# tj12323/GeoPurify

Hardware: AMD Instinct MI355X
Metric: scenes/sec (ScanNet-val shape) + pooled-feature GB/s vs HBM peak (higher is better)
Workload: dtype f32 (student convolutions and pooling: f16 hi/lo split operands, 3 MFMAs per product, fp32 accumulate)

## Files before the change

### geopurify_amd/_lib.py

```python
import ctypes
import os
from ctypes import POINTER, c_char_p, c_double, c_float, c_int32, c_int64, c_size_t, c_uint32, c_uint64, c_void_p

_HERE = os.path.dirname(os.path.abspath(__file__))
LIB_PATH = os.environ.get("GP_LIB") or os.path.join(_HERE, "libgeopurify_hip.so")

_P = c_void_p
GP_KNN_MAX_K = 127
GP_KNN_QUERY_MAX_K = 32
GP_ELEM_F32, GP_ELEM_F16, GP_ELEM_BF16 = 0, 1, 2
GP_LABEL_U8, GP_LABEL_I16, GP_LABEL_I32, GP_LABEL_I64 = 0, 1, 2, 3

SIGNATURES = {
    "gp_version": (c_int32, []),
    "gp_last_error": (c_char_p, []),
    "gp_debug_set": (c_int32, [c_int32, c_int32]),
    "gp_debug_ptr": (c_int32, [c_int32, _P, c_size_t]),
    "gp_voxelize_workspace_bytes": (c_size_t, [c_int64]),
    "gp_voxelize_f64": (c_int32, [_P, c_int64, POINTER(c_double), _P, _P, _P, _P, _P, _P, _P, c_size_t, _P]),
    "gp_fnv_hash_f64": (c_int32, [_P, c_int64, _P, _P]),
    "gp_project_points_f64": (c_int32, [_P, c_int64, POINTER(c_double), c_double, c_double, c_double,
                                        c_double, _P, c_int32, c_int32, c_int32, c_double, _P, _P, _P]),
    "gp_render_depth_f64": (c_int32, [_P, c_int64, POINTER(c_double), c_double, c_double, c_double, c_double,
                                      c_int32, c_int32, c_int32, _P, _P]),
# ... 69 lines not shown
    "gp_pool_cs_chain_flag_words": (c_size_t, [c_int64, c_int32]),
    "gp_pool_cs_chain_flag_words_d": (c_size_t, [c_int64, c_int32, c_int32]),
    "gp_pool_cs_apply_chain": (c_int32, [_P, _P, _P, _P, c_int64, _P, _P, _P, _P, _P, c_int64, c_int32, c_int32, c_int32, _P, c_int64, _P, _P, _P,
                                         c_uint32, _P]),
    "gp_lift_dense_accum": (c_int32, [_P, c_int32, c_int32, c_int32, _P, _P, _P, c_int64, _P, c_int64, _P, _P]),
    "gp_lift_dense_bilinear_accum": (c_int32, [_P, c_int32, c_int32, c_int32, c_int32, c_int32, _P, _P, _P, c_int64, _P,
                                               c_int64, _P, _P]),
    "gp_lift_dense_finish": (c_int32, [_P, c_int64, c_int32, _P, c_int64, _P, _P]),
    "gp_lift_masks_workspace_bytes": (c_size_t, [c_int32, c_int32, c_int32]),
    "gp_lift_masks_view": (c_int32, [_P, c_int32, c_int32, c_int32, _P, _P, _P, _P, _P, c_int32, c_int32,
                                     _P, _P, c_int64, _P, _P, _P, c_size_t, _P]),
    "gp_pv_count": (c_int32, [_P, c_int64, _P, _P]),
    "gp_scan_workspace_bytes": (c_size_t, [c_int64]),
    "gp_exclusive_scan_i64": (c_int32, [_P, c_int64, _P, _P, c_size_t, _P]),
    "gp_pv_fill": (c_int32, [_P, _P, c_int64, c_int32, _P, _P, _P, _P, _P]),
    "gp_segment_tables": (c_int32, [_P, c_int32, c_int32, _P, c_int32, c_float, _P, _P, _P]),
    "gp_fuse_views_top3": (c_int32, [_P, _P, _P, c_int64, _P, _P, c_int32, c_int32, c_int32, _P, c_int64, _P, _P]),
    "gp_seen_masks": (c_int32, [_P, c_int64, _P, _P, _P]),
    "gp_fuse_views_top3_fill": (c_int32, [_P, _P, _P, c_int64, _P, _P, c_int32, c_int32, c_int32, _P, _P, c_int64, _P]),
    "gp_nn1_workspace_bytes": (c_size_t, [c_int64, c_int64]),
    "gp_nn1_f64": (c_int32, [_P, c_int64, _P, c_int64, _P, _P, c_size_t, _P]),
    "gp_nn1_masked_workspace_bytes": (c_size_t, [c_int64]),
    "gp_nn1_masked_f64": (c_int32, [_P, c_int64, _P, _P, _P, _P, c_size_t, _P]),
    "gp_visible_lists_workspace_bytes": (c_size_t, [c_int64]),
    "gp_visible_lists": (c_int32, [_P, c_int64, _P, _P, _P, _P, _P, c_size_t, _P]),
    "gp_views_visible_lists_workspace_bytes": (c_size_t, [c_int64, c_int32]),
    "gp_views_visible_lists": (c_int32, [_P, c_int64, _P, _P, c_int32, c_int32, c_int32, c_int32, c_double, c_int64, c_int64,
                                         _P, _P, _P, _P, _P, _P, _P, c_size_t, _P]),
    "gp_lift_masks_views_workspace_bytes": (c_size_t, [c_int32, c_int32, c_int32, c_int32, c_int64, c_int64, c_int64]),
    "gp_lift_masks_views": (c_int32, [_P, c_int32, c_int32, c_int32, c_int32, _P, _P, _P, _P, _P, c_int32, c_int32, _P, c_int64,
                                      _P, _P, _P, _P, _P, _P, c_int32, c_int64, c_int64, _P, _P, _P, _P, _P, c_size_t, _P]),
    "gp_classify_argmax": (c_int32, [_P, c_int64, c_int32, c_int64, _P, c_int32, c_float, _P, _P, _P]),
    "gp_gather_rows_classify": (c_int32, [_P, c_int64, c_int32, _P, c_int64, _P, _P, c_int64, _P, c_int32, c_float, _P, _P, _P]),
    "gp_rows_argmax": (c_int32, [_P, c_int64, c_int32, c_int64, _P, c_int64, c_int32, _P, _P, _P]),
    "gp_col_stats_workspace_bytes": (c_size_t, [c_int64, c_int32]),
    "gp_col_stats": (c_int32, [_P, c_int64, c_int64, c_int32, _P, _P, _P, c_size_t, _P]),
    "gp_bn_train_apply": (c_int32, [_P, c_int64, c_int64, c_int32, _P, _P, _P, _P, c_float, _P, c_int64, c_int32, _P, c_int64,
                                    _P, _P, c_int64, c_float, _P, _P, _P]),
    "gp_bn_train_backward_workspace_bytes": (c_size_t, [c_int64, c_int32]),
    "gp_bn_train_backward": (c_int32, [_P, c_int64, _P, c_int64, _P, c_int64, _P, _P, c_float, _P, _P, c_int64, c_int32, _P, c_int64,
                                       _P, c_int64, _P, _P, _P, _P, _P, c_int64, _P, c_size_t, _P]),
    "gp_col_sums_f64": (c_int32, [_P, c_int64, c_int64, c_int32, _P, _P, _P, c_size_t, _P]),
    "gp_bn_bwd_sums_f64": (c_int32, [_P, c_int64, _P, c_int64, _P, c_int64, _P, _P, c_float, _P, _P, c_int64, c_int32, _P, _P, c_size_t, _P]),
    "gp_bn_bwd_apply": (c_int32, [_P, c_int64, _P, c_int64, _P, c_int64, _P, _P, c_float, _P, _P, _P, c_int64, c_int64, c_int32, _P, c_int64,
                                  _P, c_int64, _P, _P]),
    "gp_infonce_workspace_bytes": (c_size_t, [c_int64, c_int32]),
    "gp_infonce_fwd_bwd": (c_int32, [_P, c_int64, c_int64, c_int32, _P, c_int64, _P, c_int64, c_int32, c_float, _P, _P, c_int64,
                                     _P, c_size_t, _P]),
    "gp_infonce_weighted_fwd_bwd": (c_int32, [_P, c_int64, c_int64, c_int32, _P, c_int64, _P, c_int64, c_int32, c_float, _P, _P, _P, _P, c_int64,
                                              _P, c_size_t, _P]),
    "gp_conv_wgrad_workspace_bytes": (c_size_t, [c_int64, c_int32, c_int32]),
    "gp_conv_wgrad_f16x3": (c_int32, [_P, _P, c_int64, _P, _P, c_int64, _P, _P, _P, c_int64, _P, c_int32, c_int32, c_int32, c_int32,
                                      _P, _P, _P, c_size_t, _P]),
    "gp_adamw_step": (c_int32, [_P, _P, _P, _P, c_int64, c_float, c_float, c_float, c_float, c_float, c_int64, _P]),
    "gp_knn_points_f32": (c_int32, [_P, c_int64, _P, c_int64, c_int32, _P, _P, _P]),
    "gp_sampler_select": (c_int32, [_P, c_int64, c_int64, c_int64, _P, c_int32, _P, _P, _P]),
    "gp_sim_segments_f16x3": (c_int32, [_P, _P, c_int64, c_int32, _P, _P, _P, _P, c_int64, c_int64, _P, _P]),
    "gp_sampler_select_segments": (c_int32, [_P, _P, _P, _P, c_int64, c_int64, _P, c_int32, _P, _P, _P]),
    "gp_sampler_micro_segments": (c_int32, [_P, _P, _P, _P, _P, c_int64, c_int32, _P, c_int64, c_int32, _P, _P]),
    "gp_normalize_split_f16": (c_int32, [_P, c_int64, c_int32, c_int64, c_int64, c_float, _P, _P, c_int64, _P]),
    "gp_iou_hist_i64": (c_int32, [_P, _P, c_int64, c_int32, POINTER(c_int64), c_int32, _P, _P]),
    "gp_nn1_batched_workspace_bytes": (c_size_t, [c_int64]),
    "gp_nn1_batched": (c_int32, [_P, _P, _P, _P, c_int64, c_int32, _P, _P, _P, c_size_t, _P]),
    "gp_iou_hist_batched_i64": (c_int32, [_P, _P, c_int64, _P, _P, c_int64, c_int32, c_int32, POINTER(c_int64), c_int32, _P, _P]),
    "gp_sparse_conv_tiles": (c_int32, [POINTER(c_int32)]),
    "gp_segment_loss_col_step": (c_int32, []),
# ... 142 lines not shown
```

### geopurify_amd/csrc/misc.hip

```cpp
#include <cstring>
#include <rocprim/device/device_scan.hpp>

#include "gp_common.h"
#include "gp_scan_bytes.h"

namespace {

constexpr int NN_TILE = 1024;

__global__ void __launch_bounds__(256)
nn1_partial_kernel(const float *__restrict__ ref, int64_t n_ref, const float *__restrict__ qry, int64_t n_q,
                   int splits, double *__restrict__ pd, int64_t *__restrict__ pi) {
    __shared__ double sx[NN_TILE], sy[NN_TILE], sz[NN_TILE];
    int64_t q = blockIdx.x * (int64_t)blockDim.x + threadIdx.x;
    int sp = blockIdx.y;
    int64_t per = (n_ref + splits - 1) / splits;
    int64_t r0 = sp * per, r1 = r0 + per < n_ref ? r0 + per : n_ref;
    double qx = 0, qy = 0, qz = 0;
    if (q < n_q) { qx = qry[q * 3]; qy = qry[q * 3 + 1]; qz = qry[q * 3 + 2]; }
    double best = INFINITY;
    int64_t bi = -1;
    for (int64_t t0 = r0; t0 < r1; t0 += NN_TILE) {
        int64_t cnt = r1 - t0 < NN_TILE ? r1 - t0 : NN_TILE;
        __syncthreads();
// ... 320 lines not shown
    for (int j = 0; j < CL_MAXJ; ++j) {
        v[j] = (live && j < nj) ? *reinterpret_cast<const float4 *>(feat + p * ld + (j * 16 + l) * 4) : make_float4(0.f, 0.f, 0.f, 0.f);
        ss += v[j].x * v[j].x + v[j].y * v[j].y + v[j].z * v[j].z + v[j].w * v[j].w;
    }
    ss = sum16(ss);
    const float nrm = fmaxf(sqrtf(ss), 1e-12f);
    float sa = 0.f;
#pragma unroll
    for (int j = 0; j < CL_MAXJ; ++j) {
        v[j].x /= nrm; v[j].y /= nrm; v[j].z /= nrm; v[j].w /= nrm;
        sa += fabsf(v[j].x) + fabsf(v[j].y) + fabsf(v[j].z) + fabsf(v[j].w);
    }
    sa = sum16(sa);
    float bestv = -INFINITY;
    int bestc = 0;
    for (int k = 0; k < C; ++k) {
        float dot = 0.f;
#pragma unroll
        for (int j = 0; j < CL_MAXJ; ++j)
            if (j < nj) {
                const float4 t = *reinterpret_cast<const float4 *>(text + (int64_t)k * d + (j * 16 + l) * 4);
                dot += v[j].x * t.x + v[j].y * t.y + v[j].z * t.z + v[j].w * t.w;
            }
        dot = sum16(dot) * scale;
        if (dot > bestv) { bestv = dot; bestc = k; }
    }
    if (live && l == 0) {
        pred[p] = bestc;
        if (zero_row) zero_row[p] = (sa == 0.f) ? 1 : 0;
    }
}

constexpr int CL_Q = 2;
template <bool GATHER>
__global__ void __launch_bounds__(256)
classify16_lds_kernel(const float *__restrict__ feat, int64_t ld, int d, int64_t n, const float *__restrict__ text, int C,
                      float scale, int64_t *__restrict__ pred, uint8_t *__restrict__ zero_row, const int64_t *__restrict__ index,
                      const int32_t *__restrict__ row_map, float *__restrict__ out, int64_t ld_out) {
    extern __shared__ __align__(16) float cl_text[];
    for (int i = threadIdx.x * 4; i < C * d; i += 256 * 4) *reinterpret_cast<float4 *>(cl_text + i) = *reinterpret_cast<const float4 *>(text + i);
    __syncthreads();
    const int l = threadIdx.x & 15, g = threadIdx.x >> 4;
    const int nj = d / 64;
    for (int64_t base = blockIdx.x * (int64_t)(16 * CL_Q); base < n; base += (int64_t)gridDim.x * (16 * CL_Q)) {
        float4 v[CL_Q][CL_MAXJ];
        float sa[CL_Q], bestv[CL_Q];
        int bestc[CL_Q];
        bool live[CL_Q];
#pragma unroll
        for (int q = 0; q < CL_Q; ++q) {
            const int64_t p = base + g * CL_Q + q;
            live[q] = p < n;
            int64_t src_row = p;
            if constexpr (GATHER) {
                if (live[q]) { src_row = index[p]; if (row_map) src_row = row_map[src_row]; }
            }
            float ss = 0.f;
#pragma unroll
            for (int j = 0; j < CL_MAXJ; ++j) {
                v[q][j] = (live[q] && j < nj) ? *reinterpret_cast<const float4 *>(feat + src_row * ld + (j * 16 + l) * 4) : make_float4(0.f, 0.f, 0.f, 0.f);
                if constexpr (GATHER) {
                    if (live[q] && j < nj) *reinterpret_cast<float4 *>(out + p * ld_out + (j * 16 + l) * 4) = v[q][j];
                }
                ss += v[q][j].x * v[q][j].x + v[q][j].y * v[q][j].y + v[q][j].z * v[q][j].z + v[q][j].w * v[q][j].w;
            }
            ss = sum16(ss);
            const float nrm = fmaxf(sqrtf(ss), 1e-12f);
            float a = 0.f;
#pragma unroll
            for (int j = 0; j < CL_MAXJ; ++j) {
                v[q][j].x /= nrm; v[q][j].y /= nrm; v[q][j].z /= nrm; v[q][j].w /= nrm;
                a += fabsf(v[q][j].x) + fabsf(v[q][j].y) + fabsf(v[q][j].z) + fabsf(v[q][j].w);
            }
            sa[q] = sum16(a);
            bestv[q] = -INFINITY;
            bestc[q] = 0;
        }
        for (int k = 0; k < C; ++k) {
            float dot[CL_Q];
#pragma unroll
            for (int q = 0; q < CL_Q; ++q) dot[q] = 0.f;
#pragma unroll
            for (int j = 0; j < CL_MAXJ; ++j)
                if (j < nj) {
                    const float4 t = *reinterpret_cast<const float4 *>(cl_text + k * d + (j * 16 + l) * 4);
#pragma unroll
                    for (int q = 0; q < CL_Q; ++q) dot[q] += v[q][j].x * t.x + v[q][j].y * t.y + v[q][j].z * t.z + v[q][j].w * t.w;
                }
#pragma unroll
            for (int q = 0; q < CL_Q; ++q) {
                const float dv = sum16(dot[q]) * scale;
                if (dv > bestv[q]) { bestv[q] = dv; bestc[q] = k; }
            }
        }
#pragma unroll
        for (int q = 0; q < CL_Q; ++q)
            if (live[q] && l == 0) {
                const int64_t p = base + g * CL_Q + q;
                pred[p] = bestc[q];
                if (zero_row) zero_row[p] = (sa[q] == 0.f) ? 1 : 0;
            }
    }
}

constexpr int CL_WJ = 16;
__global__ void __launch_bounds__(256)
classify_wave_gather_kernel(const float *__restrict__ feat, int64_t ld, int d, int64_t n, const float *__restrict__ text, int C,
                            float scale, int64_t *__restrict__ pred, uint8_t *__restrict__ zero_row, const int64_t *__restrict__ index,
                            const int32_t *__restrict__ row_map, float *__restrict__ out, int64_t ld_out) {
    extern __shared__ __align__(16) float cl_text[];
    for (int i = threadIdx.x * 4; i < C * d; i += 256 * 4) *reinterpret_cast<float4 *>(cl_text + i) = *reinterpret_cast<const float4 *>(text + i);
    __syncthreads();
    const int lane = threadIdx.x & 63, w = threadIdx.x >> 6;
    const int nj = d / 64;
    for (int64_t base = blockIdx.x * (int64_t)(4 * CL_Q); base < n; base += (int64_t)gridDim.x * (4 * CL_Q)) {
        float u[CL_Q][CL_WJ];
        float sa[CL_Q], bestv[CL_Q];
        int bestc[CL_Q];
        bool live[CL_Q];
#pragma unroll
        for (int q = 0; q < CL_Q; ++q) {
            const int64_t p = base + w * CL_Q + q;
            live[q] = p < n;
            int64_t src_row = 0;
            if (live[q]) { src_row = index[p]; if (row_map) src_row = row_map[src_row]; }
            float ss = 0.f;
#pragma unroll
            for (int j = 0; j < CL_WJ; ++j) {
                u[q][j] = (live[q] && j < nj) ? feat[src_row * ld + j * 64 + lane] : 0.f;
                if (live[q] && j < nj) out[p * ld_out + j * 64 + lane] = u[q][j];
                ss += u[q][j] * u[q][j];
            }
            ss = gp_wave_sum(ss);
            const float nrm = fmaxf(sqrtf(ss), 1e-12f);
// ... 253 lines not shown
    } else if (fast)
        classify16_kernel<<<(int)((n * 16 + 255) / 256), 256, 0, gp_stream(stream_)>>>(feat, ld, d, n, text_norm, c, logit_scale, pred, zero_row);
    else
        classify_kernel<<<(int)((n * 64 + 255) / 256), 256, 0, gp_stream(stream_)>>>(feat, ld, d, n, text_norm, c, logit_scale,
                                                                                   pred, zero_row);
    GP_CHECK_LAUNCH();
    return GP_OK;
}

extern "C" int gp_gather_rows_classify(const float *src, int64_t ld_src, int32_t d, const int64_t *index, int64_t n, const int32_t *row_map,
                                       float *out, int64_t ld_out, const float *text_norm, int32_t c, float logit_scale, int64_t *pred,
                                       uint8_t *zero_row, void *stream_) {
    GP_CHECK_ARG(src && index && out && text_norm && pred && n > 0 && d > 0 && c > 0, "gp_gather_rows_classify: null/empty argument");
    GP_CHECK_ARG(d % 64 == 0 && d <= 64 * CL_WJ && ld_src % 4 == 0 && ld_out % 4 == 0 && ld_out >= d && (uintptr_t)src % 16 == 0 &&
                     (uintptr_t)out % 16 == 0 && (uintptr_t)text_norm % 16 == 0 && (size_t)c * d * sizeof(float) <= 64 * 1024,
                 "gp_gather_rows_classify: d=%d must be a multiple of 64 up to %d, rows 16-byte aligned, c * d * 4 <= 64 KiB (use gp_gather_rows + "
                 "gp_classify_argmax otherwise)", d, 64 * CL_WJ);
    GP_CHECK_ARG(out != src, "gp_gather_rows_classify: out must not alias src");
    if (d <= 64 * CL_MAXJ) {
        GP_SMEM_ATTR(classify16_lds_kernel<true>, 64 * 1024);
        const int64_t groups = (n + 16 * CL_Q - 1) / (16 * CL_Q);
        classify16_lds_kernel<true><<<(int)(groups < 2048 ? groups : 2048), 256, (size_t)c * d * sizeof(float), gp_stream(stream_)>>>(
            src, ld_src, d, n, text_norm, c, logit_scale, pred, zero_row, index, row_map, out, ld_out);
    } else {
        GP_SMEM_ATTR(classify_wave_gather_kernel, 64 * 1024);
        const int64_t groups = (n + 4 * CL_Q - 1) / (4 * CL_Q);
        classify_wave_gather_kernel<<<(int)(groups < 2048 ? groups : 2048), 256, (size_t)c * d * sizeof(float), gp_stream(stream_)>>>(
            src, ld_src, d, n, text_norm, c, logit_scale, pred, zero_row, index, row_map, out, ld_out);
    }
    GP_CHECK_LAUNCH();
    return GP_OK;
}

extern "C" int gp_rows_argmax(const float *logits, int64_t ld, int32_t c, int64_t n, const float *feat, int64_t ld_f,
                              int32_t d, int64_t *pred, uint8_t *zero_row, void *stream_) {
    GP_CHECK_ARG(logits && pred && n > 0 && c > 0, "gp_rows_argmax: null/empty argument");
    rows_argmax_kernel<<<(int)((n * 64 + 255) / 256), 256, 0, gp_stream(stream_)>>>(logits, ld, c, n, feat, ld_f, d, pred, zero_row);
    GP_CHECK_LAUNCH();
    return GP_OK;
}

extern "C" int gp_iou_hist_i64(const int64_t *pred, const int64_t *target, int64_t n, int32_t num_classes,
                               const int64_t *ignore_ids_host, int32_t num_ignore, int64_t *counts, void *stream_) {
    GP_CHECK_ARG(pred && target && counts && n > 0, "gp_iou_hist_i64: null/empty argument");
    GP_CHECK_ARG(num_classes > 0 && num_classes <= 4096, "gp_iou_hist_i64: num_classes=%d out of range", num_classes);
    GP_CHECK_ARG(num_ignore >= 0 && num_ignore <= 4, "gp_iou_hist_i64: at most 4 ignore ids");
    int64_t ig[4] = {0, 0, 0, 0};
    for (int i = 0; i < num_ignore; ++i) ig[i] = ignore_ids_host[i];
    int blocks = (int)((n + 255) / 256);
    if (blocks > 1024) blocks = 1024;
    iou_hist_kernel<<<blocks, 256, 3 * num_classes * sizeof(unsigned int), gp_stream(stream_)>>>(
        pred, target, n, num_classes, ig[0], ig[1], ig[2], ig[3], num_ignore,
        reinterpret_cast<unsigned long long *>(counts));
    GP_CHECK_LAUNCH();
    return GP_OK;
}
```

### geopurify_amd/ops.py

```python
import ctypes

import numpy as np
import torch

from . import _lib
from ._lib import check


def _ptr(t):
    return ctypes.c_void_p(t.data_ptr()) if t is not None else None


def _stream():
    return ctypes.c_void_p(torch.cuda.current_stream().cuda_stream)


def _ws(nbytes, device):
    return torch.empty(max(int(nbytes), 256), dtype=torch.uint8, device=device)


def _chk(t, dtype, name):
    if t.dtype != dtype or not t.is_cuda or not t.is_contiguous():
        raise ValueError(f"{name}: expected contiguous CUDA {dtype}, got {t.dtype} cuda={t.is_cuda} contig={t.is_contiguous()}")
    return t
# ... 230 lines not shown
    rinv = torch.empty(nv, dtype=torch.float32, device=dev)
    sc = torch.empty(2, dtype=torch.float32, device=dev) if want_scale else None
    ws = _ws(256, dev) if want_scale else None
    check(lib.gp_voxel_rows_operands(_ptr(f), f.stride(0), int(d), _ptr(geo), geo.stride(0), int(dg), _ptr(order), _ptr(seg_start), int(nv),
                                     _ptr(row_map), _ptr(X), X.stride(0), int(cin_pad), _ptr(rows), rows.stride(0), _ptr(rinv), _ptr(sc),
                                     _ptr(ws), ws.numel() if ws is not None else 0, _stream()), "gp_voxel_rows_operands")
    return X, (rows, None, rinv), sc


def gather_rows(src, d, index, out=None, row_map=None):
    lib = _lib.load()
    n = index.shape[0]
    if out is None:
        out = torch.empty((n, d), dtype=torch.float32, device=src.device)
    check(lib.gp_gather_rows(_ptr(src), src.stride(0), int(d), _ptr(index), n, _ptr(row_map), _ptr(out),
                             out.stride(0), _stream()), "gp_gather_rows")
    return out


def gather_rows_classify(src, d, index, text_norm, logit_scale, row_map=None):
    lib = _lib.load()
    n = index.shape[0]
    out = torch.empty((n, d), dtype=torch.float32, device=src.device)
    pred = torch.empty(n, dtype=torch.int64, device=src.device)
    zero = torch.empty(n, dtype=torch.uint8, device=src.device)
    check(lib.gp_gather_rows_classify(_ptr(src), src.stride(0), int(d), _ptr(index), n, _ptr(row_map), _ptr(out), out.stride(0),
                                      _ptr(text_norm), int(text_norm.shape[0]), float(logit_scale), _ptr(pred), _ptr(zero), _stream()),
          "gp_gather_rows_classify")
    return out, pred, zero


def can_gather_rows_classify(d, num_classes):
    return d % 64 == 0 and d <= 1024 and num_classes * d * 4 <= 64 * 1024


def pool_cs_width_ok(d):
    return d % 256 == 0 and 256 <= d <= 1024


def sparse_conv(x, nbr_map, w, scale=None, shift=None, residual=None, relu=False, out=None):
    lib = _lib.load()
    nv = x.shape[0]
    if w.dim() == 3:
        kv, cin, cout = w.shape
    else:
        kv, (cin, cout) = 1, w.shape
    _chk(w, torch.float32, "w")
    if out is None:
        out = torch.empty((nv, cout), dtype=torch.float32, device=x.device)
    check(lib.gp_sparse_conv(_ptr(x), x.stride(0), _ptr(nbr_map) if kv > 1 else None, nv, _ptr(w), int(kv),
                             int(cin), int(cout), _ptr(scale), _ptr(shift), _ptr(residual),
                             residual.stride(0) if residual is not None else 0, int(bool(relu)), _ptr(out),
                             out.stride(0), _stream()), "gp_sparse_conv")
    return out


class ConvPairs:

    def __init__(self, pair_in, pair_pos, seg_off, tile_start, nseg, num_pairs, nv):
        self.pair_in, self.pair_pos, self.pair_off, self.tile_start = pair_in, pair_pos, seg_off, tile_start
        self.nseg, self.num_pairs, self.nv = nseg, num_pairs, nv
        self.partial = None
        self.num_chunks, self.chunk_row_off, self.chunk_tile_off, self.chunk_pair_off = 0, None, None, None

    def _set_chunks(self, rows, tiles, pairs):
        n = len(rows) - 1
# ... 2286 lines not shown
```

### geopurify_amd/pipeline.py

```python
from dataclasses import dataclass, field
from typing import List, Optional

import numpy as np
import torch

from . import ops
from .bicubic import aa_bicubic_taps

GEO_DIM = 6
CONV_PAD = 32


def _pad_to(v, m):
    return (v + m - 1) // m * m


class StudentWeights:

    def __init__(self, state_dict, device, eps=1e-5, mode="f16x3", residual_from_planes=True, interleaved_rows=True, blocked_weights=True,
                 head="f16x3"):
        sd = {k: v.detach() for k, v in state_dict.items()}
        self.mode = mode
        self.residual_from_planes = bool(residual_from_planes)
        self.interleaved_rows = bool(interleaved_rows)
# ... 124 lines not shown


@dataclass
class SceneBatch:
    scene_coords: torch.Tensor
    scene_coords_3d: torch.Tensor
    scene_inds_reconstruct: torch.Tensor
    scene_label: torch.Tensor
    scene_gauss_features: torch.Tensor
    views: List[ViewLists] = field(default_factory=list)
    order: Optional[torch.Tensor] = None
    seg_start: Optional[torch.Tensor] = None
    extent: Optional[list] = None
    imgs: Optional[torch.Tensor] = None
    ent: Optional[dict] = None

    def as_tuple(self):
        dev = self.scene_coords.device
        N = self.scene_coords.shape[0]
        e = torch.empty(0, device=dev)
        V = len(self.views)
        ori = torch.cat([torch.cat([torch.full((len(v.pt), 1), float(i), device=dev),
                                    self.scene_coords[v.pt]], 1) for i, v in enumerate(self.views)]) if V else e
        mask = torch.zeros((V, N), dtype=torch.long, device=dev)
        for i, v in enumerate(self.views):
            mask[i, v.pt] = 1
        vid = torch.arange(V, device=dev).repeat_interleave(N)
        mask_2ds = torch.stack([vid, mask.reshape(-1)], 1)
        xl = torch.cat([v.x for v in self.views]) if V else e.long()
        yl = torch.cat([v.y for v in self.views]) if V else e.long()
        imgs = self.imgs if self.imgs is not None else e
        return (self.scene_coords, self.scene_coords_3d, self.scene_inds_reconstruct, self.scene_label, ori,
                e, e, e, e, e, e, imgs, xl, yl, mask_2ds, e, e, e, (None,) * V, self.scene_gauss_features)


def _view_matrices(cfg, views):
    from .synthetic import mapper_intrinsics
    out = []
    for v in views:
        K = mapper_intrinsics(cfg, v.K)
        if cfg.dataset == "scannet":
            w2c = np.asarray(v.pose).T.astype(np.float64)
        else:
            w2c = np.linalg.inv(np.asarray(v.pose))
        out.append((w2c, K))
    return out


def _voxel_extent(vox):
    ci = vox["coords_aug"].to(torch.int32)
    return ops.minmax_i32(ci.contiguous())[3:6].to(torch.int64) + 1


def build_scene_batch(scene, rigid, device="cuda", val_keep=10_000_000, batch_views=True, mark=None):
    from .synthetic import mapper_intrinsics
    cfg = scene.cfg
    dev = torch.device(device)
    coords64 = scene.coords_dev if hasattr(scene, "coords_dev") else torch.from_numpy(scene.coords).to(dev)
    N = coords64.shape[0]
    vox = ops.voxelize(coords64, rigid)
    if mark is not None:
        mark("voxelize")
    W, H = cfg.image_dim
    V = len(scene.views)
    gauss = scene.gauss_dev if hasattr(scene, "gauss_dev") else torch.from_numpy(
        np.concatenate([scene.colors, scene.normals], 1).astype(np.float32)).to(dev)
# ... 116 lines not shown
        if (cs_ok or mfma_ok) and num_iters >= 3 and D in (256, 512, 768):
            return "cs" if cs_ok else "mfma"
        return "tiles" if tiles_ok else "ell"
    if family in ("cs", "chain"):
        if not cs_ok:
            raise ValueError(f"pool_mode='{mode}' needs D in (256, 512, 768, 1024) and K <= 96 (D={D}, K={K})")
        return "chain" if family == "chain" and num_iters >= 2 else "cs"
    if family in ("mfma", "mfma_persist") and not mfma_ok:
        raise ValueError(f"pool_mode='mfma' needs D == 512 and block_rows*K <= 16384 (D={D}, K={K})")
    if family == "tiles" and not tiles_ok:
        return "ell"
    return family


class HotPath:

    def __init__(self, student: StudentWeights, mask_shape, K=96, sharpen=20.0, num_iters=19, device="cuda",
                 pool_mode="auto", pool_tile_rows=8, pool_block_rows=64, batch_views=True, pool_structure_ahead=True, affinity_mfma=True,
                 all_views_max_pairs=2e11, pool_row_order="rcb"):
        self.student = student
        self.batch_views = batch_views
        self.all_views_max_pairs = float(all_views_max_pairs)
        self.pool_mode, self.pool_tile_rows, self.pool_block_rows = _known_pool_mode(pool_mode), pool_tile_rows, pool_block_rows
        self.pool_structure_ahead = bool(pool_structure_ahead)
        self.affinity_mfma = bool(affinity_mfma)
        self.pool_row_order = pool_row_order
        self.mask_shape = tuple(mask_shape)
        self.K, self.sharpen, self.num_iters = K, sharpen, num_iters
        self.device = torch.device(device)
        self._taps = {}
        self.stats = {}
        self.stage_mark = None
        self._chain_ops = []
        self.keep_lifted, self.last_lifted = False, None

    def _tap_tables(self, h, w):
        key = (h, w)
        if key not in self._taps:
            H, W = self.mask_shape
            tx0, twx = aa_bicubic_taps(w, W)
            ty0, twy = aa_bicubic_taps(h, H)
            d = self.device
            self._taps[key] = tuple(torch.from_numpy(a).to(d) for a in (tx0, twx, ty0, twy))
        return self._taps[key]

    def lift_masks(self, batch: SceneBatch, vlm):
        dev = self.device
        N = batch.scene_coords.shape[0]
        V = len(batch.views)
        has_img = batch.imgs is not None and batch.imgs.numel() > 0
        batched = ((not has_img or getattr(vlm, "ignores_image", False)) and torch.is_tensor(getattr(vlm, "mask_embed", None))
                   and vlm.mask_embed.dim() == 3 and vlm.mask_embed.is_contiguous())
        outs = None
        if batched:
            text_embed, logit_scale = vlm.text_embed, float(vlm.logit_scale)
            Q, D = vlm.mask_embed.shape[1:]
        else:
            outs = [vlm(v.src_view, image=batch.imgs[v.src_view]) if has_img else vlm(v.src_view) for v in batch.views]
            if V:
                text_embed, logit_scale = outs[0]["text_embed"].to(dev), float(outs[0]["logit_scale"])
                Q, D = outs[0]["mask_embed"].shape
            else:
                text_embed, logit_scale = vlm.text_embed, float(vlm.logit_scale)
                Q, D = 1, text_embed.shape[1]
        text_norm = torch.nn.functional.normalize(text_embed, dim=-1).contiguous()
        C = text_norm.shape[0]
# ... 64 lines not shown
        cnt = torch.zeros(N, dtype=torch.float32, device=dev)
        for v in batch.views:
            ops.lift_dense_accum(vlm.feat[v.src_view], v.pt, v.x, v.y, s, cnt)
        seen = ops.lift_dense_finish(s, D, cnt)
        nn = ops.nn1_masked(batch.scene_coords, seen, 1 - seen)
        src = torch.where(nn >= 0, nn, torch.arange(N, device=dev))
        return ops.gather_rows(s, D, src), vlm.text_embed, vlm.logit_scale

    def lift_lseg(self, batch: SceneBatch, vlm: LSegFeatureVLM):
        dev = self.device
        N = batch.scene_coords.shape[0]
        D = vlm.feat_lo.shape[1]
        H, W = vlm.image_shape
        s = torch.zeros((N, D), dtype=torch.float32, device=dev)
        cnt = torch.zeros(N, dtype=torch.float32, device=dev)
        for v in batch.views:
            ops.lift_dense_bilinear_accum(vlm.feat_lo[v.src_view], H, W, v.pt, v.x, v.y, s, cnt)
        seen = ops.lift_dense_finish(s, D, cnt)
        nn = ops.nn1_masked(batch.scene_coords, seen, 1 - seen)
        src = torch.where(nn >= 0, nn, torch.arange(N, device=dev))
        return ops.gather_rows(s, D, src), vlm.text_embed, vlm.logit_scale

    def prepare(self, batch: SceneBatch, F):
        dev = self.device
        N, D = F.shape
        st = self.student
        assert st.cin == D + GEO_DIM, f"student expects {st.cin} input channels, lift gives {D}+{GEO_DIM}"
        coords = batch.scene_coords_3d.floor().to(torch.int32).contiguous()
        Nv = coords.shape[0]
        perm, rank = ops.morton_order(coords)
        cs = coords[perm.long()].contiguous()
        mark = self.stage_mark if self.stage_mark is not None else (lambda name: None)
        mark("morton order")
        if batch.order is None:
            order = torch.sort(batch.scene_inds_reconstruct, stable=True).indices
            segc = torch.zeros(Nv + 1, dtype=torch.int64, device=dev)
            segc[1:] = torch.bincount(batch.scene_inds_reconstruct, minlength=Nv).cumsum(0)
            batch.order, batch.seg_start = order, segc
        family = self._pool_family(D)
        xs = sc = None
        if st.one_pass_input(F, batch.scene_gauss_features):
            X, xs, sc = ops.voxel_rows_operands(F, D, batch.scene_gauss_features, GEO_DIM, batch.order, batch.seg_start, Nv, st.cin_pad,
                                                row_map=rank, want_scale=family in ("cs", "chain"))
        else:
            X = torch.zeros((Nv, st.cin_pad), dtype=torch.float32, device=dev)
            ops.scatter_mean_csr(F, D, batch.order, batch.seg_start, Nv, X, col0=0, row_map=rank)
            ops.scatter_mean_csr(batch.scene_gauss_features, GEO_DIM, batch.order, batch.seg_start, Nv, X, col0=D,
                                 row_map=rank)
        mark("scatter_mean")
        if batch.extent is not None:
            grid = ops.grid_build(cs, [0, 0, 0], batch.extent)
        else:
            grid = ops.grid_build(cs)
        nbr_map = ops.kernel_map_build(grid, cs)
        pairs = ops.conv_pairs_build(nbr_map, col_tiles=max(1, st.hidden // 256)) if any(l[0] == "f16x3" for l in st.layers) else None
        mark("grid+kernel_map")
        nbr = ops.knn_lattice(grid, cs, perm, self.K)
        mark("kNN")
        state = {"X": X, "rank": rank, "nbr_map": nbr_map, "pairs": pairs, "nbr": nbr, "Nv": Nv, "D": D, "pool": None,
                 "xs": xs if xs is not None else st.split_input(X)}
        if family in ("cs", "chain"):
            if sc is None:
                sc = ops.pow2_scale(X, D)
            how = self.pool_structure_ahead
            if how and self.affinity_mfma and self.K <= 96 and self.student is not None and self.student.embed == 128:
                how = "valid"
            rho = None
            nbr_op = nbr
            if how == "valid" and self.pool_row_order == "rcb" and Nv > 1024:
                sigma, rho = ops.rcb_order(cs, 1024, 128)
                nbr_op = ops.rows_renumber(nbr, sigma, rho)
                state["rank_pool"] = rho[rank.long()].contiguous()
            state["pool"] = {"op": ops.pool_cs_plan(nbr_op, structure=how), "sc": sc, "rho": rho, "nbr": nbr_op,
                             "x_split": ops.split_f16(X, D, scale=sc[0:1], dst_row=rho),
                             "pong": tuple(torch.empty((Nv, D), dtype=torch.float16, device=dev) for _ in range(2))}
            if family == "chain" and (state["pool"]["op"].dst is not None or state["pool"]["op"].valid is not None):
                ops.pool_cs_deps(state["pool"]["op"], D)
            mark("pool plan+split")
        return state

    def refine(self, batch: SceneBatch, F, after_student=None, prepared=None, classify_text=None):
        p = prepared if prepared is not None else self.prepare(batch, F)
        X, rank, nbr, Nv, D = p["X"], p["rank"], p["nbr"], p["Nv"], p["D"]
        mark = self.stage_mark if self.stage_mark is not None else (lambda name: None)
        op = p["pool"]["op"] if p["pool"] is not None else None
        mfma_aff = op is not None and op.valid is not None
        rho = p["pool"]["rho"] if (p["pool"] is not None and mfma_aff) else None
        E = self.student.forward(X, p["nbr_map"], p["pairs"], x_split=p.get("xs"), mark=self.stage_mark, planes=mfma_aff, plane_rows=rho)
        mark("embed head" if self.stage_mark is not None else "student")
        if after_student is not None:
            after_student()
        if mfma_aff:
            ops.affinity_cs_fragments(None, self.sharpen, op, planes=E)
            w = None
        else:
            w = ops.affinity_softmax(E, nbr, self.sharpen, into=op if op is not None and op.dst is not None else None)
        mark("affinity")
        self._last_E, self._last_E_rho = E, rho
        self._last_pool_inputs = (X, nbr, w, Nv, D)
        self._last_pool_plan = p["pool"]
        out = self._pool(X, nbr, w, Nv, D, plan=p["pool"])
        mark("pooling")
        self._fused_pred = None
        if classify_text is not None and ops.can_gather_rows_classify(D, classify_text[0].shape[0]) and classify_text[0].shape[0] <= 32:
            text_norm = torch.nn.functional.normalize(classify_text[0], dim=-1).contiguous()
            out, pred, zero = ops.gather_rows_classify(out, D, batch.scene_inds_reconstruct, text_norm, classify_text[1],
                                                       row_map=p.get("rank_pool", rank))
            self._fused_pred = (out, classify_text[0], pred, zero)
        else:
            out = ops.gather_rows(out, D, batch.scene_inds_reconstruct, row_map=p.get("rank_pool", rank))
        mark("gather")
        self.stats = {"Nv": Nv, "nbr_map": p["nbr_map"], "pool_bytes_per_iter": Nv * (2 * D * 4 + self.K * 8),
                      "pool_kernel": self._pool_kernel}
        return out

    def _pool_family(self, D):
        return resolve_pool_mode(self.pool_mode, D, self.K, self.num_iters, self.pool_tile_rows, self.pool_block_rows)

    def _pool(self, X, nbr, w, Nv, D, plan=None):
        dev = X.device
        family = self._pool_family(D)
        if w is None and (plan is None or not plan["op"].filled):
            E = self._last_E
            if isinstance(E, tuple):
                E = (E[0].float() + E[1].float()) / ops.AFFINITY_PLANE_SCALE
                if getattr(self, "_last_E_rho", None) is not None:
                    E = E[self._last_E_rho.long()]
            w = ops.affinity_softmax(E.contiguous(), nbr, self.sharpen)
        if self.num_iters == 0:
            out = torch.empty((Nv, D), dtype=torch.float32, device=dev)
            out.copy_(X[:, :D])
            self._pool_kernel = "none"
            return out
        if family in ("cs", "chain"):
            if plan is None:
                sc = ops.pow2_scale(X, D)
                plan = {"op": ops.pool_cs_plan(nbr), "sc": sc, "x_split": ops.split_f16(X, D, scale=sc[0:1]),
                        "pong": tuple(torch.empty((Nv, D), dtype=torch.float16, device=dev) for _ in range(2))}
            op = plan["op"] if plan["op"].filled else ops.pool_cs_fill(plan["op"], nbr, w)
            out = torch.empty((Nv, D), dtype=torch.float32, device=dev)
            sc = plan["sc"]
            sp = [plan["x_split"], plan["pong"]]
            if self.stage_mark is not None:
                self.stage_mark("pool operator fill")
            if family == "chain":
                if op.dep is None:
                    ops.pool_cs_deps(op, D)
# ... 124 lines not shown
```

### include/geopurify_hip.h

```cpp
#ifndef GEOPURIFY_HIP_H
#define GEOPURIFY_HIP_H

#include <stddef.h>
#include <stdint.h>

#ifdef __cplusplus
extern "C" {
#endif

#define GP_OK 0
#define GP_EINVAL (-22)
#define GP_ENOMEM (-12)
#define GP_EHIP (-5)
#define GP_ERANGE (-34)

#define GP_KNN_MAX_K 127

#define GP_ELEM_F32 0
#define GP_ELEM_F16 1
#define GP_ELEM_BF16 2

int gp_version(void);
int gp_debug_set(int32_t key, int32_t value);
int gp_debug_ptr(int32_t key, void *device_buffer, size_t bytes);
// ... 202 lines not shown
size_t gp_scan_workspace_bytes(int64_t n);
int gp_exclusive_scan_i64(const int64_t *in, int64_t n, int64_t *out, void *workspace,
                          size_t workspace_bytes, void *stream);
int gp_pv_fill(const int64_t *pt, const int32_t *seg, int64_t n_v, int32_t view,
               const int64_t *pv_start, int32_t *cursor, int32_t *pv_view, int32_t *pv_seg,
               void *stream);
int gp_fuse_views_top3(const int64_t *pv_start, const int32_t *pv_view, const int32_t *pv_seg,
                       int64_t n, const float *f_seg, const float *logit_seg, int32_t q, int32_t d,
                       int32_t c, float *out, int64_t ld_out, uint8_t *seen, void *stream);
int gp_seen_masks(const int64_t *pv_start, int64_t n, uint8_t *seen, uint8_t *unseen, void *stream);
int gp_fuse_views_top3_fill(const int64_t *pv_start, const int32_t *pv_view, const int32_t *pv_seg,
                            int64_t n, const float *f_seg, const float *logit_seg, int32_t q, int32_t d,
                            int32_t c, const int64_t *nn, float *out, int64_t ld_out, void *stream);
size_t gp_nn1_workspace_bytes(int64_t n_ref, int64_t n_query);
int gp_nn1_f64(const float *ref_xyz, int64_t n_ref, const float *query_xyz, int64_t n_query,
               int64_t *nn, void *workspace, size_t workspace_bytes, void *stream);
size_t gp_nn1_masked_workspace_bytes(int64_t n);
int gp_nn1_masked_f64(const float *xyz, int64_t n, const uint8_t *ref_mask, const uint8_t *query_mask,
                      int64_t *nn, void *workspace, size_t workspace_bytes, void *stream);
size_t gp_visible_lists_workspace_bytes(int64_t n);
int gp_visible_lists(const int64_t *mapping, int64_t n, int64_t *pt, int64_t *x, int64_t *y,
                     int64_t *count_dev, void *workspace, size_t workspace_bytes, void *stream);
size_t gp_views_visible_lists_workspace_bytes(int64_t n, int32_t nviews);
int gp_views_visible_lists(const double *coords, int64_t n, const double *params, const double *depth, int32_t nviews,
                           int32_t width, int32_t height, int32_t cut_bound, double vis_thres, int64_t min_visible,
                           int64_t val_keep, int64_t *ent_pt, int64_t *ent_x, int64_t *ent_y, int32_t *ent_view,
                           int64_t *view_off, uint8_t *keep, void *workspace, size_t workspace_bytes, void *stream);

int gp_classify_argmax(const float *feat, int64_t ld, int32_t d, int64_t n, const float *text_norm,
                       int32_t c, float logit_scale, int64_t *pred, uint8_t *zero_row, void *stream);
int gp_gather_rows_classify(const float *src, int64_t ld_src, int32_t d, const int64_t *index, int64_t n, const int32_t *row_map,
                            float *out, int64_t ld_out, const float *text_norm, int32_t c, float logit_scale, int64_t *pred,
                            uint8_t *zero_row, void *stream);
int gp_rows_argmax(const float *logits, int64_t ld, int32_t c, int64_t n, const float *feat, int64_t ld_f,
                   int32_t d, int64_t *pred, uint8_t *zero_row, void *stream);
int gp_iou_hist_i64(const int64_t *pred, const int64_t *target, int64_t n, int32_t num_classes,
                    const int64_t *ignore_ids_host, int32_t num_ignore, int64_t *counts,
                    void *stream);
size_t gp_nn1_batched_workspace_bytes(int64_t nv);
int gp_nn1_batched(const uint64_t *keys_sorted, const int32_t *ids, const uint8_t *ref_mask, const uint8_t *query_mask, int64_t nv,
                   int32_t axes, int32_t *nn, int32_t *status, void *workspace, size_t workspace_bytes, void *stream);
int gp_iou_hist_batched_i64(const int64_t *pred, const int32_t *coords, int64_t rows, const int64_t *target, const int64_t *index,
                            int64_t n, int32_t num_batches, int32_t num_classes, const int64_t *ignore_ids_host, int32_t num_ignore,
                            int64_t *counts, void *stream);
int32_t gp_segment_loss_col_step(void);
int gp_segment_loss_unit_rows(const float *y, int64_t ld_y, int32_t d, int64_t n, float *u, int64_t ld_u, int32_t d_pad, uint8_t *zero,
                              void *stream);
size_t gp_segment_loss_items_workspace_bytes(int64_t n, int64_t p);
int gp_segment_loss_items(const int32_t *coords, const uint8_t *zero, int64_t n, const int64_t *labels, const int64_t *index, int64_t p,
                          int32_t c, const int64_t *ignore_ids_host, int32_t num_ignore, int32_t reduction, uint8_t *row_valid,
                          int64_t *item_off, int32_t *item_id, int64_t *entry_cnt, float *entry_w, int64_t *status, void *workspace,
                          size_t workspace_bytes, void *stream);
int gp_segment_loss_rows(const float *z, int64_t ld_z, int64_t r, int32_t c, int32_t c_pad, const int32_t *coords, const uint8_t *row_valid,
                         const int64_t *item_off, const int32_t *item_id, const int64_t *labels, const float *entry_w, float *g,
                         int64_t ld_g, float *lse, double *term, void *stream);
size_t gp_segment_loss_reduce_workspace_bytes(int64_t n, int32_t num_entries);
int gp_segment_loss_reduce(const double *term, const int32_t *coords, int64_t n, const int64_t *entry_cnt, int32_t num_entries,
                           int32_t reduction, float *loss, float *per_entry, void *workspace, size_t workspace_bytes, void *stream);

size_t gp_col_stats_workspace_bytes(int64_t nv, int32_t c);
int gp_col_stats(const float *y, int64_t ld, int64_t nv, int32_t c, float *mean, float *var,
                 void *workspace, size_t workspace_bytes, void *stream);
int gp_bn_train_apply(const float *y, int64_t ld, int64_t nv, int32_t c, const float *mean, const float *var,
                      const float *gamma, const float *beta, float eps, const float *residual, int64_t ld_res,
                      int32_t relu, float *out, int64_t ld_out, void *out_hi, void *out_lo, int64_t ld_split,
                      float momentum, float *running_mean, float *running_var, void *stream);
// ... 254 lines not shown
```

Before: 46.90.

## Classify pooled voxels once per voxel via CSR and scatter to points

Adds a CSR-driven gather+classify kernel that loads each voxel's pooled feature once, normalises it and scores it against the text embeddings once, then writes the row and prediction to every point in that voxel. Previously each point re-read and re-classified its voxel's feature. The pipeline now builds and reuses the voxel-to-points CSR and uses the new path when shapes allow. It also caches the normalised text embeddings across calls, keyed on tensor identity and version. Load balance depends on points per voxel, and the scattered writes to point rows are irregular.

```diff
diff --git a/geopurify_amd/_lib.py b/geopurify_amd/_lib.py
--- a/geopurify_amd/_lib.py
+++ b/geopurify_amd/_lib.py
@@ -125,6 +125,7 @@
                                       _P, _P, _P, _P, _P, _P, c_int32, c_int64, c_int64, _P, _P, _P, _P, _P, c_size_t, _P]),
     "gp_classify_argmax": (c_int32, [_P, c_int64, c_int32, c_int64, _P, c_int32, c_float, _P, _P, _P]),
     "gp_gather_rows_classify": (c_int32, [_P, c_int64, c_int32, _P, c_int64, _P, _P, c_int64, _P, c_int32, c_float, _P, _P, _P]),
+    "gp_gather_rows_classify_csr": (c_int32, [_P, c_int64, c_int32, _P, _P, c_int64, _P, _P, c_int64, _P, c_int32, c_float, _P, _P, _P]),
     "gp_rows_argmax": (c_int32, [_P, c_int64, c_int32, c_int64, _P, c_int64, c_int32, _P, _P, _P]),
     "gp_col_stats_workspace_bytes": (c_size_t, [c_int64, c_int32]),
     "gp_col_stats": (c_int32, [_P, c_int64, c_int64, c_int32, _P, _P, _P, c_size_t, _P]),
diff --git a/geopurify_amd/csrc/misc.hip b/geopurify_amd/csrc/misc.hip
--- a/geopurify_amd/csrc/misc.hip
+++ b/geopurify_amd/csrc/misc.hip
@@ -376,6 +376,45 @@
 }
 
 constexpr int CL_Q = 2;
+
+__device__ __forceinline__ float cl16_normalise(float4 (&v)[CL_MAXJ]) {
+    float ss = 0.f;
+#pragma unroll
+    for (int j = 0; j < CL_MAXJ; ++j) ss += v[j].x * v[j].x + v[j].y * v[j].y + v[j].z * v[j].z + v[j].w * v[j].w;
+    ss = sum16(ss);
+    const float nrm = fmaxf(sqrtf(ss), 1e-12f);
+    float a = 0.f;
+#pragma unroll
+    for (int j = 0; j < CL_MAXJ; ++j) {
+        v[j].x /= nrm; v[j].y /= nrm; v[j].z /= nrm; v[j].w /= nrm;
+        a += fabsf(v[j].x) + fabsf(v[j].y) + fabsf(v[j].z) + fabsf(v[j].w);
+    }
+    return sum16(a);
+}
+template <int Q>
+__device__ __forceinline__ void cl16_classes(const float4 (&v)[Q][CL_MAXJ], const float *cl_text, int C, int d, int nj, int l, float scale,
+                                             float (&bestv)[Q], int (&bestc)[Q]) {
+#pragma unroll
+    for (int q = 0; q < Q; ++q) { bestv[q] = -INFINITY; bestc[q] = 0; }
+    for (int k = 0; k < C; ++k) {
+        float dot[Q];
+#pragma unroll
+        for (int q = 0; q < Q; ++q) dot[q] = 0.f;
+#pragma unroll
+        for (int j = 0; j < CL_MAXJ; ++j)
+            if (j < nj) {
+                const float4 t = *reinterpret_cast<const float4 *>(cl_text + k * d + (j * 16 + l) * 4);
+#pragma unroll
+                for (int q = 0; q < Q; ++q) dot[q] += v[q][j].x * t.x + v[q][j].y * t.y + v[q][j].z * t.z + v[q][j].w * t.w;
+            }
+#pragma unroll
+        for (int q = 0; q < Q; ++q) {
+            const float dv = sum16(dot[q]) * scale;
+            if (dv > bestv[q]) { bestv[q] = dv; bestc[q] = k; }
+        }
+    }
+}
+
 template <bool GATHER>
 __global__ void __launch_bounds__(256)
 classify16_lds_kernel(const float *__restrict__ feat, int64_t ld, int d, int64_t n, const float *__restrict__ text, int C,
@@ -399,44 +438,16 @@
             if constexpr (GATHER) {
                 if (live[q]) { src_row = index[p]; if (row_map) src_row = row_map[src_row]; }
             }
-            float ss = 0.f;
 #pragma unroll
             for (int j = 0; j < CL_MAXJ; ++j) {
                 v[q][j] = (live[q] && j < nj) ? *reinterpret_cast<const float4 *>(feat + src_row * ld + (j * 16 + l) * 4) : make_float4(0.f, 0.f, 0.f, 0.f);
                 if constexpr (GATHER) {
                     if (live[q] && j < nj) *reinterpret_cast<float4 *>(out + p * ld_out + (j * 16 + l) * 4) = v[q][j];
                 }
-                ss += v[q][j].x * v[q][j].x + v[q][j].y * v[q][j].y + v[q][j].z * v[q][j].z + v[q][j].w * v[q][j].w;
-            }
-            ss = sum16(ss);
-            const float nrm = fmaxf(sqrtf(ss), 1e-12f);
-            float a = 0.f;
-#pragma unroll
-            for (int j = 0; j < CL_MAXJ; ++j) {
-                v[q][j].x /= nrm; v[q][j].y /= nrm; v[q][j].z /= nrm; v[q][j].w /= nrm;
-                a += fabsf(v[q][j].x) + fabsf(v[q][j].y) + fabsf(v[q][j].z) + fabsf(v[q][j].w);
-            }
-            sa[q] = sum16(a);
-            bestv[q] = -INFINITY;
-            bestc[q] = 0;
-        }
-        for (int k = 0; k < C; ++k) {
-            float dot[CL_Q];
-#pragma unroll
-            for (int q = 0; q < CL_Q; ++q) dot[q] = 0.f;
-#pragma unroll
-            for (int j = 0; j < CL_MAXJ; ++j)
-                if (j < nj) {
-                    const float4 t = *reinterpret_cast<const float4 *>(cl_text + k * d + (j * 16 + l) * 4);
-#pragma unroll
-                    for (int q = 0; q < CL_Q; ++q) dot[q] += v[q][j].x * t.x + v[q][j].y * t.y + v[q][j].z * t.z + v[q][j].w * t.w;
-                }
-#pragma unroll
-            for (int q = 0; q < CL_Q; ++q) {
-                const float dv = sum16(dot[q]) * scale;
-                if (dv > bestv[q]) { bestv[q] = dv; bestc[q] = k; }
-            }
-        }
+            }
+            sa[q] = cl16_normalise(v[q]);
+        }
+        cl16_classes<CL_Q>(v, cl_text, C, d, nj, l, scale, bestv, bestc);
 #pragma unroll
         for (int q = 0; q < CL_Q; ++q)
             if (live[q] && l == 0) {
@@ -444,6 +455,61 @@
                 pred[p] = bestc[q];
                 if (zero_row) zero_row[p] = (sa[q] == 0.f) ? 1 : 0;
             }
+    }
+}
+
+constexpr int CLV_T = 512;
+constexpr int CLV_SWEEP = CLV_T / 16;
+constexpr int CLV_WG_PER_CU = 3;
+struct ClvMeta {
+    int64_t s, e;
+    int row;
+};
+__global__ void __launch_bounds__(CLV_T, 2 * CLV_WG_PER_CU)
+classify16_csr_kernel(const float *__restrict__ feat, int64_t ld, int d, int64_t nv, const int64_t *__restrict__ order,
+                      const int64_t *__restrict__ seg_start, const int32_t *__restrict__ row_map, const float *__restrict__ text, int C,
+                      float scale, float *__restrict__ out, int64_t ld_out, int64_t *__restrict__ pred, uint8_t *__restrict__ zero_row) {
+    extern __shared__ __align__(16) float cl_text[];
+    for (int i = threadIdx.x * 4; i < C * d; i += CLV_T * 4) *reinterpret_cast<float4 *>(cl_text + i) = *reinterpret_cast<const float4 *>(text + i);
+    __syncthreads();
+    const int l = threadIdx.x & 15, g = threadIdx.x >> 4;
+    const int nj = d / 64;
+    const int64_t stride = (int64_t)gridDim.x * CLV_SWEEP;
+    auto load_meta = [&](int64_t vx, ClvMeta &m) {
+        m.s = m.e = 0; m.row = 0;
+        if (vx < nv) {
+            m.s = seg_start[vx];
+            m.e = seg_start[vx + 1];
+            m.row = row_map ? row_map[vx] : (int)vx;
+        }
+    };
+    ClvMeta m, mn;
+    int64_t vx = blockIdx.x * (int64_t)CLV_SWEEP + g;
+    load_meta(vx, m);
+    for (int64_t base = blockIdx.x * (int64_t)CLV_SWEEP; base < nv; base += stride, vx += stride) {
+        const int cnt = (int)(m.e - m.s);
+        float4 v[1][CL_MAXJ];
+#pragma unroll
+        for (int j = 0; j < CL_MAXJ; ++j)
+            v[0][j] = (cnt > 0 && j < nj) ? *reinterpret_cast<const float4 *>(feat + (int64_t)m.row * ld + (j * 16 + l) * 4) : make_float4(0.f, 0.f, 0.f, 0.f);
+        const int64_t p0 = cnt > 0 ? order[m.s] : 0;
+        load_meta(vx + stride, mn);
+        for (int i = 0; i < cnt; ++i) {
+            const int64_t p = i == 0 ? p0 : order[m.s + i];
+#pragma unroll
+            for (int j = 0; j < CL_MAXJ; ++j)
+                if (j < nj) *reinterpret_cast<float4 *>(out + p * ld_out + (j * 16 + l) * 4) = v[0][j];
+        }
+        float bestv[1];
+        int bestc[1];
+        const float sa = cl16_normalise(v[0]);
+        cl16_classes<1>(v, cl_text, C, d, nj, l, scale, bestv, bestc);
+        for (int i = l; i < cnt; i += 16) {
+            const int64_t p = i == 0 ? p0 : order[m.s + i];
+            pred[p] = bestc[0];
+            if (zero_row) zero_row[p] = (sa == 0.f) ? 1 : 0;
+        }
+        m = mn;
     }
 }
 
@@ -763,6 +829,27 @@
     return GP_OK;
 }
 
+extern "C" int gp_gather_rows_classify_csr(const float *src, int64_t ld_src, int32_t d, const int64_t *order, const int64_t *seg_start,
+                                           int64_t nv, const int32_t *row_map, float *out, int64_t ld_out, const float *text_norm, int32_t c,
+                                           float logit_scale, int64_t *pred, uint8_t *zero_row, void *stream_) {
+    GP_CHECK_ARG(src && order && seg_start && out && text_norm && pred && nv > 0 && d > 0 && c > 0,
+                 "gp_gather_rows_classify_csr: null/empty argument");
+    GP_CHECK_ARG(nv < ((int64_t)1 << 31), "gp_gather_rows_classify_csr: nv=%lld voxels, more than 2^31-1", (long long)nv);
+    GP_CHECK_ARG(d % 64 == 0 && d <= 64 * CL_MAXJ && ld_src % 4 == 0 && ld_out % 4 == 0 && ld_out >= d && (uintptr_t)src % 16 == 0 &&
+                     (uintptr_t)out % 16 == 0 && (uintptr_t)text_norm % 16 == 0 && (size_t)c * d * sizeof(float) <= 64 * 1024,
+                 "gp_gather_rows_classify_csr: d=%d must be a multiple of 64 up to %d, rows 16-byte aligned, c * d * 4 <= 64 KiB (use "
+                 "gp_gather_rows_classify otherwise)", d, 64 * CL_MAXJ);
+    GP_CHECK_ARG(out != src, "gp_gather_rows_classify_csr: out must not alias src");
+    GP_SMEM_ATTR(classify16_csr_kernel, 64 * 1024);
+    const int64_t sweeps = (nv + CLV_SWEEP - 1) / CLV_SWEEP;
+    const int cu = gp_cu_count();
+    const int64_t cap = (int64_t)(cu > 0 ? cu : 256) * CLV_WG_PER_CU;
+    classify16_csr_kernel<<<(int)(sweeps < cap ? sweeps : cap), CLV_T, (size_t)c * d * sizeof(float), gp_stream(stream_)>>>(
+        src, ld_src, d, nv, order, seg_start, row_map, text_norm, c, logit_scale, out, ld_out, pred, zero_row);
+    GP_CHECK_LAUNCH();
+    return GP_OK;
+}
+
 extern "C" int gp_rows_argmax(const float *logits, int64_t ld, int32_t c, int64_t n, const float *feat, int64_t ld_f,
                               int32_t d, int64_t *pred, uint8_t *zero_row, void *stream_) {
     GP_CHECK_ARG(logits && pred && n > 0 && c > 0, "gp_rows_argmax: null/empty argument");
diff --git a/geopurify_amd/ops.py b/geopurify_amd/ops.py
--- a/geopurify_amd/ops.py
+++ b/geopurify_amd/ops.py
@@ -286,6 +286,36 @@
 
 def can_gather_rows_classify(d, num_classes):
     return d % 64 == 0 and d <= 1024 and num_classes * d * 4 <= 64 * 1024
+
+
+def gather_rows_classify_csr(src, d, order, seg_start, text_norm, logit_scale, row_map=None, out=None, pred=None, zero=None):
+    lib = _lib.load()
+    if src.dtype != torch.float32 or src.dim() != 2 or src.stride(1) != 1:
+        raise ValueError(f"gather_rows_classify_csr: src must be f32 [rows, >= d] with unit column stride, got {src.dtype} {list(src.shape)}")
+    _chk(order, torch.int64, "order")
+    _chk(seg_start, torch.int64, "seg_start")
+    n, nv = order.shape[0], seg_start.shape[0] - 1
+    if order.dim() != 1 or seg_start.dim() != 1 or nv < 1 or nv > src.shape[0]:
+        raise ValueError(f"gather_rows_classify_csr: order [n] and seg_start [nv + 1] with nv <= {src.shape[0]} rows expected, got "
+                         f"{list(order.shape)} / {list(seg_start.shape)}")
+    if row_map is not None and (_chk(row_map, torch.int32, "row_map").dim() != 1 or row_map.shape[0] < nv):
+        raise ValueError(f"gather_rows_classify_csr: row_map must be i32 [{nv}], got {list(row_map.shape)}")
+    if out is None:
+        out = torch.empty((n, d), dtype=torch.float32, device=src.device)
+    if pred is None:
+        pred = torch.empty(n, dtype=torch.int64, device=src.device)
+    if zero is None:
+        zero = torch.empty(n, dtype=torch.uint8, device=src.device)
+    if out.shape[0] != n or pred.shape != (n,) or zero.shape != (n,) or pred.dtype != torch.int64 or zero.dtype != torch.uint8:
+        raise ValueError(f"gather_rows_classify_csr: out [{n}, >= {d}] f32, pred [{n}] i64 and zero [{n}] u8 expected")
+    check(lib.gp_gather_rows_classify_csr(_ptr(src), src.stride(0), int(d), _ptr(order), _ptr(seg_start), nv, _ptr(row_map), _ptr(out),
+                                          out.stride(0), _ptr(text_norm), int(text_norm.shape[0]), float(logit_scale), _ptr(pred),
+                                          _ptr(zero), _stream()), "gp_gather_rows_classify_csr")
+    return out, pred, zero
+
+
+def can_gather_rows_classify_csr(d, num_classes):
+    return d % 64 == 0 and d <= 512 and num_classes * d * 4 <= 64 * 1024
 
 
 def pool_cs_width_ok(d):
diff --git a/geopurify_amd/pipeline.py b/geopurify_amd/pipeline.py
--- a/geopurify_amd/pipeline.py
+++ b/geopurify_amd/pipeline.py
@@ -180,6 +180,15 @@
         imgs = self.imgs if self.imgs is not None else e
         return (self.scene_coords, self.scene_coords_3d, self.scene_inds_reconstruct, self.scene_label, ori,
                 e, e, e, e, e, e, imgs, xl, yl, mask_2ds, e, e, e, (None,) * V, self.scene_gauss_features)
+
+
+def voxel_points_csr(batch, nv):
+    if batch.order is None or batch.seg_start is None:
+        index = batch.scene_inds_reconstruct
+        seg = torch.zeros(nv + 1, dtype=torch.int64, device=index.device)
+        seg[1:] = torch.bincount(index, minlength=nv).cumsum(0)
+        batch.order, batch.seg_start = torch.sort(index, stable=True).indices, seg
+    return batch.order, batch.seg_start
 
 
 def _view_matrices(cfg, views):
@@ -362,6 +371,7 @@
         self.stats = {}
         self.stage_mark = None
         self._chain_ops = []
+        self._text_norm = None
         self.keep_lifted, self.last_lifted = False, None
 
     def _tap_tables(self, h, w):
@@ -492,11 +502,7 @@
         cs = coords[perm.long()].contiguous()
         mark = self.stage_mark if self.stage_mark is not None else (lambda name: None)
         mark("morton order")
-        if batch.order is None:
-            order = torch.sort(batch.scene_inds_reconstruct, stable=True).indices
-            segc = torch.zeros(Nv + 1, dtype=torch.int64, device=dev)
-            segc[1:] = torch.bincount(batch.scene_inds_reconstruct, minlength=Nv).cumsum(0)
-            batch.order, batch.seg_start = order, segc
+        voxel_points_csr(batch, Nv)
         family = self._pool_family(D)
         xs = sc = None
         if st.one_pass_input(F, batch.scene_gauss_features):
@@ -563,9 +569,15 @@
         mark("pooling")
         self._fused_pred = None
         if classify_text is not None and ops.can_gather_rows_classify(D, classify_text[0].shape[0]) and classify_text[0].shape[0] <= 32:
-            text_norm = torch.nn.functional.normalize(classify_text[0], dim=-1).contiguous()
-            out, pred, zero = ops.gather_rows_classify(out, D, batch.scene_inds_reconstruct, text_norm, classify_text[1],
-                                                       row_map=p.get("rank_pool", rank))
+            text_norm = self._unit_text(classify_text[0])
+            N = batch.scene_inds_reconstruct.shape[0]
+            if (ops.can_gather_rows_classify_csr(D, text_norm.shape[0]) and batch.order is not None and batch.seg_start is not None
+                    and batch.order.shape[0] == N and batch.seg_start.shape[0] == Nv + 1):
+                out, pred, zero = ops.gather_rows_classify_csr(out, D, batch.order, batch.seg_start, text_norm, classify_text[1],
+                                                               row_map=p.get("rank_pool", rank))
+            else:
+                out, pred, zero = ops.gather_rows_classify(out, D, batch.scene_inds_reconstruct, text_norm, classify_text[1],
+                                                           row_map=p.get("rank_pool", rank))
             self._fused_pred = (out, classify_text[0], pred, zero)
         else:
             out = ops.gather_rows(out, D, batch.scene_inds_reconstruct, row_map=p.get("rank_pool", rank))
@@ -573,6 +585,15 @@
         self.stats = {"Nv": Nv, "nbr_map": p["nbr_map"], "pool_bytes_per_iter": Nv * (2 * D * 4 + self.K * 8),
                       "pool_kernel": self._pool_kernel}
         return out
+
+    def _unit_text(self, text):
+        c = self._text_norm
+        if c is None or c[0] is not text or c[1] != text._version:
+            t = torch.nn.functional.normalize(text, dim=-1).contiguous()
+            c = self._text_norm = (text, text._version, t, torch.cuda.current_stream().record_event() if t.is_cuda else None)
+        elif c[3] is not None:
+            torch.cuda.current_stream().wait_event(c[3])
+        return c[2]
 
     def _pool_family(self, D):
         return resolve_pool_mode(self.pool_mode, D, self.K, self.num_iters, self.pool_tile_rows, self.pool_block_rows)
diff --git a/include/geopurify_hip.h b/include/geopurify_hip.h
--- a/include/geopurify_hip.h
+++ b/include/geopurify_hip.h
@@ -258,6 +258,9 @@
 int gp_gather_rows_classify(const float *src, int64_t ld_src, int32_t d, const int64_t *index, int64_t n, const int32_t *row_map,
                             float *out, int64_t ld_out, const float *text_norm, int32_t c, float logit_scale, int64_t *pred,
                             uint8_t *zero_row, void *stream);
+int gp_gather_rows_classify_csr(const float *src, int64_t ld_src, int32_t d, const int64_t *order, const int64_t *seg_start, int64_t nv,
+                                const int32_t *row_map, float *out, int64_t ld_out, const float *text_norm, int32_t c, float logit_scale,
+                                int64_t *pred, uint8_t *zero_row, void *stream);
 int gp_rows_argmax(const float *logits, int64_t ld, int32_t c, int64_t n, const float *feat, int64_t ld_f,
                    int32_t d, int64_t *pred, uint8_t *zero_row, void *stream);
 int gp_iou_hist_i64(const int64_t *pred, const int64_t *target, int64_t n, int32_t num_classes,
```

New measurement: 47.12 (median of 6 runs). No clear change (+0.5%).
